# JuliaMolSim/Molly.jl

Hardware: AMD Instinct MI355X
Metric: ns_per_day (higher is better)
Workload: dtype f32; 1 GPU; 1M-atom LJ fluid (argon, rho=21.1/nm3), cubic PBC, DistanceCutoff 1.0 nm, r_list 1.2 nm, dt 2 fs, VelocityVerlet, remove_CM_motion=1; integrator=vv, n_atoms=1000000, rebuild_every=10, parallelism=single domain, block_atoms=256, j_split=2, pairs_half_list=75841147

## Files before the change

molly.jl_amd/csrc/engine.hip:

```cpp
#include <algorithm>
#include <chrono>
#include <cstddef>
#include <cstdlib>
#include <cstring>
#include <limits>
#include <memory>
#include <new>
#include <string>
#include <vector>

#include <unistd.h>

#include "bonded.h"
#include "stochastic.h"
#include "constraints.h"
#include "virtual_sites.h"
#include "pme.h"
#include "step_fused.h"
#include "hilbert.h"
#include "kernels.h"
#include "list_policy.h"
#include "replan.h"
#include "halo_step.h"
#include "forces_launch.h"
// ... 102 lines not shown
        MHIP_HIP(hipEventRecord(ev[st][used[st]].second, s));
        if (++used[st] >= 8192) resolve(s);
    }
    void resolve(hipStream_t s) {
        MHIP_HIP(hipStreamSynchronize(s));
        for (int st = 0; st < NS; ++st) {
            for (size_t k = 0; k < used[st]; ++k) { float t = 0; MHIP_HIP(hipEventSynchronize(ev[st][k].second)); MHIP_HIP(hipEventElapsedTime(&t, ev[st][k].first, ev[st][k].second)); ms[st] += t; ++calls[st]; }
            used[st] = 0;
        }
    }
    void reset() { for (int st = 0; st < NS; ++st) { used[st] = 0; ms[st] = 0; calls[st] = 0; } }
    void reserve(int st, size_t n) { while (ev[st].size() < n) add(st); }
    void add(int st) { Event a, b; a.make(); b.make(); ev[st].emplace_back(std::move(a), std::move(b)); }
};

static int env_int(const char* name, int dflt) { const char* v = std::getenv(name); return v && *v ? std::atoi(v) : dflt; }


template <class T> class Engine final : public EngineBase {
    using T4 = typename Vec<T>::T4;
    using T2 = typename Vec<T>::T2;

    mhip_config cfg;
    GridP<T> G;
    InterP<T> I;
    int ljm = LJ_OFF, coulm = MHIP_COUL_NONE;
    int64_t cap, n_owned, n_ghost, n_tot;
    Stream stream;
    int device = 0;

    DBuf<T4> pos[2], vel[2], frc[2]; DBuf<T2> lj[2]; DBuf<int32_t> orig[2]; DBuf<int32_t> inv;
    int cur = 0;
    DBuf<uint32_t> key_in, key_out, cell_rank; DBuf<int32_t> idx_in, perm, cell_cnt, cell_start; DBuf<unsigned char> cub_tmp;
    bool hilbert_ok = true;
    DBuf<int32_t> xl_start; DBuf<uint32_t> xl_list; bool has_exc = false; int xl_span = 0; int64_t n_special = 0;
    static constexpr int X_CAP = 32;
    static constexpr int MAX_THREADS = BlockLimits<T>::max_threads;
    int BI = 256, JS = 1, n_blocks = 0, T_cap = 0, R_cap = 0, C_cap = 0, max_tile = 0, max_rows = 0;
    int ljm_base = LJ_OFF;
    int eshift = 0;
    bool scaled_entries_off = false;
    int want_eshift() const {
        return (!scaled_entries_off && std::is_same<T, float>::value && ljm == LJ_DIST_UNIFORM && coulm == MHIP_COUL_NONE && n_special == 0 && !tri_mode && !G.no_list) ? ESHIFT_SCALED : 0;
    }
    int slot_cap() const { return ((want_eshift() ? SLOT_MAX_SCALED : TILE_SLOT_MAX) - 1) & ~3; }
    DBuf<int32_t> tile_idx, tile_cnt, wave_rows; DBuf<uint2> nbr; DBuf<T4> blk_center;
    DBuf<int32_t> wave_rows_in, tile_idx_in, tile_cnt_in, rows_x, tile_idx_x, tile_cnt_x; DBuf<uint2> nbr_in, nbr_x; DBuf<T4> pos_snap; DBuf<float> blk_disp2; int max_tile_in = 0;
    bool inner_valid = false, prune_disp_exceeded = false;
    DBuf<uint16_t> cnt_in, cnt_outer; bool cnt_outer_valid = false;
    DBuf<uint2> nbr_gs; DBuf<int32_t> rows_gs; DBuf<T4> frc_parts; int64_t gs_list_id = -1;
    bool inner_is_outer = false; const bool adopt_env = env_int("MOLLYHIP_ADOPT_OUTER", 1) != 0; int64_t n_adopted = 0;
    const int gs_env = env_int("MOLLYHIP_GROUP_SPLIT", -1);
    int gs_groups() const {
        if (!std::is_same<T, float>::value || ljm != LJ_DIST || !(coulm == MHIP_COUL_REACTION_FIELD || (coulm == MHIP_COUL_EWALD_DIRECT && I.approx_erfc))) return 0;
        if (!dual || tri_mode || n_ghost > 0 || G.no_list || gs_env == 0) return 0;
        const int want = gs_env > 0 ? gs_env : 4;
        if (want != 4 || JS % want != 0 || BI * (JS / want) != 256) return 0;
        if (gs_env < 0 && (int64_t)n_blocks * JS * (BI / WAVE) > 2 * 4096) return 0;
        if ((int64_t)n_blocks * want > 16384) return 0;
        return want;
    }
    DBuf<int32_t> blk_ghost, blk_ghost_in; bool ghost_flags_ok = false, ghost_flags_in_ok = false;
    bool interior_done = false;
    int64_t pass_step = 0;
    DBuf<T4> pos_snap_in;
    ListPolicy lp = [] { ListPolicy p; p.inner_skin_fixed = env_int("MOLLYHIP_INNER_SKIN_FIXED", 0) != 0; return p; }();
// ... 26 lines not shown
    DBuf<T> stage_a, stage_b; DBuf<int32_t> stage_i;
    Bonded<T> bonded;
    Pme<T> pme; double pc_sum = 0, pc_abs2_sum = 0; bool pc_valid = false;
    DBuf<T4> frc_side; const T4* pend_a = nullptr;

    bool stale = true, minimg = false, params_set = false, state_set = false, frc_valid = false;
    bool coords_moved = false, export_needs_search = false; int64_t n_set_state_refresh = 0;
    int64_t last_build_step = std::numeric_limits<int64_t>::min();
    int64_t n_rebuilds = 0, n_force_calls = 0, n_gs_passes = 0; double last_rebuild_ms = 0;
    PassPlan last_plan;
    Prof prof;
    const bool trace_on = env_int("MOLLYHIP_DEBUG", 0) >= 2;
    const bool debug_on = env_int("MOLLYHIP_DEBUG", 0) == 1 || env_int("MOLLYHIP_DEBUG", 0) >= 3;
    void tr(const char* what) {
        if (!trace_on) return;
        (void)hipStreamSynchronize(stream);
        std::fprintf(stderr, "[mhip %d] %s (n_owned %lld n_ghost %lld BI %d JS %d T_cap %d R_cap %d)\n", (int)getpid(), what, (long long)n_owned, (long long)n_ghost, BI, JS, T_cap, R_cap);
        std::fflush(stderr);
    }

  public:
    explicit Engine(const mhip_config& c) : cfg(c) {
        cap = c.n_atoms; n_owned = cap; n_ghost = 0; n_tot = cap;
        if (cap <= 0) throw ApiError{MHIP_ERR_INVALID, "n_atoms must be positive"};
        if (cap > (int64_t)1 << 30) throw ApiError{MHIP_ERR_INVALID, "n_atoms too large for int32 indexing"};
        int ndev = 0;
        if (hipGetDeviceCount(&ndev) != hipSuccess || ndev <= 0) throw ApiError{MHIP_ERR_NO_DEVICE, "no HIP device visible (libmollyhip has no CPU fallback)"};
        device = c.device_id;
        if (device < 0 || device >= ndev) throw ApiError{MHIP_ERR_INVALID, "device_id out of range"};
        MHIP_HIP(hipSetDevice(device));
        stream.create(hipStreamNonBlocking);
        setup_inter(); setup_grid();
        for (int k = 0; k < 2; ++k) { pos[k].reserve(cap); vel[k].reserve(cap); frc[k].reserve(cap); lj[k].reserve(cap); orig[k].reserve(cap); }
        inv.reserve(cap); key_in.reserve(cap); key_out.reserve(cap); idx_in.reserve(cap); perm.reserve(cap);
        flags.reserve(N_FLAGS); red_out.reserve(8); vcm.reserve(4); cm_step.reserve(2 * 4 * 1024);
        h_flags.make(N_FLAGS); h_red.make(8);
        for (int k = 0; k < 2; ++k) { MHIP_HIP(hipMemsetAsync(pos[k].p, 0, cap * sizeof(T4), stream)); MHIP_HIP(hipMemsetAsync(vel[k].p, 0, cap * sizeof(T4), stream)); MHIP_HIP(hipMemsetAsync(frc[k].p, 0, cap * sizeof(T4), stream)); MHIP_HIP(hipMemsetAsync(lj[k].p, 0, cap * sizeof(T2), stream)); }
        std::vector<int32_t> iota(cap); for (int64_t i = 0; i < cap; ++i) iota[i] = (int32_t)i;
        MHIP_HIP(hipMemcpyAsync(orig[0].p, iota.data(), cap * sizeof(int32_t), hipMemcpyHostToDevice, stream));
        MHIP_HIP(hipMemcpyAsync(inv.p, iota.data(), cap * sizeof(int32_t), hipMemcpyHostToDevice, stream));
        MHIP_HIP(hipStreamSynchronize(stream));
        size_t tb = 0; MHIP_HIP(sort_pairs_u32(nullptr, tb, key_in.p, key_out.p, idx_in.p, perm.p, (int)cap, 32, stream));
        size_t tb2 = 0; MHIP_HIP(exclusive_sum_i32(nullptr, tb2, cell_cnt.p, cell_start.p, 2 * G.ncell + 1, stream));
        cub_tmp.reserve(std::max(tb, tb2) + 256);
        choose_blocking();
    }
    ~Engine() override {
        (void)hipSetDevice(device);
        if (stream) (void)hipStreamSynchronize(stream);
    }

  private:
    void setup_inter() {
        const mhip_interactions& p = cfg.inter;
        std::memset(&I, 0, sizeof(I));
        I.lj = p.lj_enabled; I.lj_cut = p.lj_cutoff_kind; I.lj_rc = T(p.lj_rc); I.lj_rc2 = I.lj_rc * I.lj_rc; I.lj_ra = T(p.lj_ra); I.lj_w = T(p.lj_weight_special);
        I.coul = p.coul_kind; I.coul_cut = p.coul_cutoff_kind; I.c_rc = T(p.coul_rc); I.c_rc2 = I.c_rc * I.c_rc; I.c_ra = T(p.coul_ra);
        I.ke = T(p.coul_ke); I.c_w = T(p.coul_weight_special); I.alpha = T(p.ewald_alpha); I.approx_erfc = p.ewald_approx_erfc;
        I.two_over_sqrt_pi = T(2) / std::sqrt(T(M_PI));
        if (p.lj_cutoff_kind < 0 || p.lj_cutoff_kind > 5 || p.coul_cutoff_kind < 0 || p.coul_cutoff_kind > 5 || p.coul_kind < 0 || p.coul_kind > 3)
            throw ApiError{MHIP_ERR_INVALID, "unknown cutoff / coulomb kind"};
        if (p.coul_kind == MHIP_COUL_REACTION_FIELD) {
            T rc = I.c_rc, rc3 = rc * rc * rc, e = T(p.rf_dielectric);
            if (std::isinf(p.rf_dielectric)) { I.krf = T(1) / (T(2) * rc3); I.crf = T(3) * (T(1) / (T(2) * rc)); }
            else { I.krf = (T(1) / rc3) * (e - T(1)) / (T(2) * e + T(1)); I.crf = (T(1) / rc) * (T(3) * e) / (T(2) * e + T(1)); }
        }
        ljm = !p.lj_enabled ? LJ_OFF : (p.lj_cutoff_kind == MHIP_CUTOFF_DISTANCE ? LJ_DIST : LJ_GENERIC);
// ... 182 lines not shown
        if (!pending_cm.mode()) return;
        hipLaunchKernelGGL(k_shift_vel<T>, dim3(std::min(cdiv(n_owned, 256), 1024)), dim3(256), 0, stream, n_owned, vel[cur].p, (const T*)vcm.p,
                           pending_cm.parts_arg(), pending_cm.n, vs_on ? (const int32_t*)orig[cur].p : nullptr, (const uint8_t*)vs_flag.p);
        pending_cm.none();
    }

    const T* to_device(const void* host_or_dev, size_t count, int mem_kind, DBuf<T>& stage) {
        if (!host_or_dev) return nullptr;
        if (mem_kind == MHIP_MEM_DEVICE) return (const T*)host_or_dev;
        stage.reserve(count);
        MHIP_HIP(hipMemcpyAsync(stage.p, host_or_dev, count * sizeof(T), hipMemcpyHostToDevice, stream));
        return stage.p;
    }

    void rebuild(int64_t step_n) {
        try { rebuild_impl(step_n); }
        catch (const ApiError& e) {
            if (e.code != MHIP_ERR_CAPACITY || !dual) throw;
            if (n_ghost > 0 || ghost_margin > 0 || host_prune) dual_disabled = true;
            else if (lp.outer_margin > 0.06) ++margin_halvings; else if (!margin_zero) margin_zero = true; else dual_disabled = true;
            if (debug_on) std::fprintf(stderr, "[mhip] dual list %s (capacity): %s\n", dual_disabled ? "off" : (margin_zero ? "without outer margin" : "margin halved"), e.msg.c_str());
            regrid();
            rebuild(step_n);
        }
    }

    void rebuild_impl(int64_t step_n) {
        lp.next_check_step = -1;
        const int sub_bits = (ilog2(2 * G.ncell + 1) + 1 + 6 <= 32) ? 6 : 0;
        if (!params_set || !state_set) throw ApiError{MHIP_ERR_STATE, "set_atoms and set_state must be called before forces"};
        auto t0 = std::chrono::steady_clock::now();
        const int o = cur, n = 1 - cur;
        const int ncell2 = 2 * G.ncell + 1;
        prof.begin(3, stream);
        const int nb256 = cdiv(n_tot, 256);
        MHIP_HIP(hipMemsetAsync(cell_cnt.p, 0, (size_t)ncell2 * sizeof(int32_t), stream));
        tr("k_cell_keys");
        hipLaunchKernelGGL(k_cell_keys<T>, dim3(nb256), dim3(256), 0, stream, n_tot, n_owned, (const T4*)pos[o].p, (const int32_t*)inv.p,
                           (const uint32_t*)cell_rank.p, key_in.p, idx_in.p, cell_cnt.p, G, sub_bits);
        tr("sort_pairs");
        size_t tb = cub_tmp.n;
        MHIP_HIP(sort_pairs_u32(cub_tmp.p, tb, key_in.p, key_out.p, idx_in.p, perm.p, (int)n_tot, std::min(32, ilog2(2 * G.ncell + 1) + 1 + sub_bits), stream));
        tb = cub_tmp.n;
        MHIP_HIP(exclusive_sum_i32(cub_tmp.p, tb, cell_cnt.p, cell_start.p, ncell2, stream));
        tr("k_permute");
        hipLaunchKernelGGL(k_permute<T>, dim3(nb256), dim3(256), 0, stream, n_tot, (const int32_t*)perm.p, (const T4*)pos[o].p, (const T4*)vel[o].p,
                           (const T4*)frc[o].p, (const T2*)lj[o].p, (const int32_t*)orig[o].p, pos[n].p, vel[n].p, frc[n].p, lj[n].p, orig[n].p, inv.p);
        prof.end(3, stream);
        cur = n;
        if (n_ghost > 0 && has_exc) throw ApiError{MHIP_ERR_UNSUPPORTED, "exclusion lists with ghost atoms are not supported"};
        if (tri_mode && !tri_grid && n_tot + 8 > TILE_SLOT_MAX) throw ApiError{MHIP_ERR_UNSUPPORTED, "a TriclinicBoundary whose cell heights allow no cell grid (fewer than 6 cells of r_list/2 on every axis) is limited to 32 759 atoms"};

        for (int attempt = 0; attempt < 12; ++attempt) {
            n_blocks = cdiv(n_owned, BI);
            bool walk = !G.no_list && (!tri_mode || tri_grid);
            size_t lds = build_lds_bytes(T_cap, BI, C_cap, walk);
            if (walk && !tri_grid && lds > (size_t)MAX_LDS_BYTES) { walk = false; lds = build_lds_bytes(T_cap, BI, C_cap, false); }
            if (lds > (size_t)MAX_LDS_BYTES) {
                if (BI > 64) { BI /= 2; JS = std::min(JS * 2, MAX_THREADS / BI); estimate_capacities(); continue; }
                throw ApiError{MHIP_ERR_CAPACITY, "neighbourhood tile of one 64-atom block does not fit the 160 KiB LDS (r_list too large for this density): T_cap " + std::to_string(T_cap) +
                               " C_cap " + std::to_string(C_cap) + " bytes " + std::to_string(lds)};
            }
            tile_idx.reserve((size_t)n_blocks * T_cap); tile_cnt.reserve(n_blocks); wave_rows.reserve((size_t)n_blocks * JS * (BI / WAVE));
            nbr.reserve((size_t)n_blocks * JS * R_cap * BI); blk_center.reserve(n_blocks);
            MHIP_HIP(hipMemsetAsync(flags.p, 0, N_FLAGS * sizeof(int32_t), stream));
            BuildArgs<T> A;
            A.G = G; A.n_owned = n_owned; A.n_tot = n_tot; A.BI = BI; A.BI_shift = ilog2(BI); A.JS = JS; A.T_cap = T_cap; A.R_cap = R_cap; A.C_cap = C_cap;
            A.pos = pos[cur].p; A.orig = orig[cur].p; A.cell_start = cell_start.p; A.cell_rank = cell_rank.p;
            A.xl_start = has_exc ? xl_start.p : nullptr; A.xl_list = xl_list.p; A.xl_span = xl_span; A.X_cap = X_CAP;
            A.tile_idx = tile_idx.p; A.tile_cnt = tile_cnt.p; A.nbr = nbr.p; A.wave_rows = wave_rows.p; A.blk_center = blk_center.p; A.flags = flags.p;
            A.margin = G.no_list ? T(0) : G.r_list * T(1e-3);
            A.approx = dual ? 1 : 0;
            A.walk = walk ? 1 : 0;
            A.eshift = eshift = want_eshift();
            A.cnt_out = nullptr; cnt_outer_valid = false;
            A.dbg = stamps_begin((size_t)n_blocks * 16 * 8);
            if (gs_groups() > 0 && adopt_env) { cnt_outer.reserve((size_t)n_blocks * JS * BI); A.cnt_out = cnt_outer.p; cnt_outer_valid = true; }
            prof.begin(1, stream);
            tr("k_build");
            auto go = [&](auto kern) { set_lds_limit(kern, lds); hipLaunchKernelGGL(kern, dim3(n_blocks), dim3(BI * JS), lds, stream, A); };
            if (A.walk && !A.xl_start) { if (A.approx) go(k_build<T, true, true, false>); else go(k_build<T, true, false, false>); }
            else if (A.walk) { if (A.approx) go(k_build<T, true, true>); else go(k_build<T, true, false>); }
            else { if (A.approx) go(k_build<T, false, true>); else go(k_build<T, false, false>); }
            hipLaunchKernelGGL(k_build_summary, dim3(std::min(64, cdiv(n_blocks * JS * (BI / WAVE), 256))), dim3(256), 0, stream, n_blocks, n_blocks * JS * (BI / WAVE), R_cap, (const int32_t*)tile_cnt.p, wave_rows.p, (const float*)nullptr, flags.p);
            prof.end(1, stream);
            MHIP_HIP(hipGetLastError());
            MHIP_HIP(hipMemcpyAsync(h_flags, flags.p, N_FLAGS * sizeof(int32_t), hipMemcpyDeviceToHost, stream));
            MHIP_HIP(hipStreamSynchronize(stream));
            if (A.dbg) stamps_dump(".build", (size_t)n_blocks * 16 * 8);
            int ovf = h_flags[FLAG_OVERFLOW];
            if (!ovf) break;
            if (ovf & OVF_SLOT) {
                if (eshift) { scaled_entries_off = true; estimate_capacities(); continue; }
                if (BI > 64) { BI /= 2; JS = std::min(JS * 2, MAX_THREADS / BI); estimate_capacities(); continue; }
                throw ApiError{MHIP_ERR_CAPACITY, "more atoms within r_list of one 64-atom block than a 16-bit list entry can name"};
            }
            if (ovf & OVF_BOXCELLS) {
                if (h_flags[FLAG_MAX_CELLS] <= MAX_BOX_CELLS) { C_cap = std::min<int>(MAX_BOX_CELLS, (int)(h_flags[FLAG_MAX_CELLS] * 1.1) + 8); continue; }
                if (BI > 64) { BI /= 2; JS = std::min(JS * 2, MAX_THREADS / BI); estimate_capacities(); continue; }
                throw ApiError{MHIP_ERR_CAPACITY, "block neighbourhood spans more than 8192 cells"};
            }
            if (ovf & OVF_TILE) T_cap = std::min<int>(slot_cap(), (((int)(h_flags[FLAG_MAX_TILE] * 1.15) + 32) + 3) & ~3);
            if (ovf & OVF_ROWS) R_cap = (int)(h_flags[FLAG_MAX_ROWS] * 1.2) + 4;
            if (attempt == 11) throw ApiError{MHIP_ERR_CAPACITY, "neighbour structures did not converge"};
        }
        minimg = h_flags[FLAG_MINIMG] != 0;
        max_tile = h_flags[FLAG_MAX_TILE]; max_rows = h_flags[FLAG_MAX_ROWS]; total_rows = outer_rows = h_flags[FLAG_TOTAL_ROWS];
        last_plan = PassPlan{}; plan_tile(last_plan, pass_shape(false, 0, false, PassReq{}), max_tile);
        throw_capacity(last_plan);
        red_part.reserve(std::max<size_t>(7 * (size_t)n_blocks, 4 * (size_t)cdiv(n_owned, 256)) + 8);
        bonded.on_reorder();
        ++n_outer; lp.last_outer_step = step_n;
        if (dual) {
            pos_snap.reserve(cap);
            MHIP_HIP(hipMemcpyAsync(pos_snap.p, pos[cur].p, (size_t)n_tot * sizeof(T4), hipMemcpyDeviceToDevice, stream));
            inner_valid = false; inner_is_outer = false; prune_disp_exceeded = false; ghost_flags_in_ok = false;
            if (lp.cur_dt > 0 && lp.skin_in < lp.skin && !host_prune) {
                (void)max_disp2_since(pos_snap);
                const double drift = lp.drift_ahead(0.0, 1, rebuild_every());
                if (lp.grow_inner_skin(drift, n_ghost > 0)) inner_skin_grown(drift);
            }
        }
        if (lazy_single) {
            pos_snap_in.reserve(cap);
// ... 2259 lines not shown
```

molly.jl_amd/csrc/kernels.h:

```cpp
#pragma once
#include <type_traits>
#include "pass_plan.h"
#include "physics.h"
#include "halo_xfer.h"
#include "philox.h"
#include "thermostat_step.h"

namespace mhip {

enum { FLAG_MINIMG = 0, FLAG_OVERFLOW = 1, FLAG_MAX_TILE = 2, FLAG_MAX_ROWS = 3, FLAG_NAN = 4, FLAG_TOTAL_ROWS = 5, FLAG_MAX_CELLS = 6, FLAG_MAX_DISP2 = 7, FLAG_MAX_V2 = 8, N_FLAGS = 10 };
enum { OVF_TILE = 1, OVF_ROWS = 2, OVF_BOXCELLS = 4, OVF_SLOT = 8 };

constexpr int MAX_BOX_CELLS = 8192;
constexpr uint32_t XL_EXCLUDED = 1u << 30, XL_SPECIAL = 1u << 31, XL_INDEX = (1u << 30) - 1u;

constexpr int SLOT_MAX_SCALED = 16383;
__host__ __device__ inline uint32_t entry_slot(uint32_t e, int sh) { return sh ? (e >> sh) : (e & 0x7fffu); }
__host__ __device__ inline uint32_t entry_special(uint32_t e, int sh) { return sh ? 0u : (e >> 15); }
__host__ __device__ inline uint32_t make_entry(uint32_t slot, uint32_t sp, int sh) { return sh ? (slot << sh) : (slot | (sp << 15)); }

template <class T> __device__ inline int cell_coord(T x, int d, const GridP<T>& G) {
    T rel = G.periodic[d] ? x : x - G.origin[d];
    int c = (int)M<T>::floor(rel * G.inv_cs[d]);
    return min(max(c, 0), G.nc[d] - 1);
}

extern "C" __device__ int mhip_writelane_i32(int src, int lane, int old) __asm("llvm.amdgcn.writelane.i32");
__device__ inline void mask_to_lane(int& lo, int& hi, unsigned long long mask, int dst) {
    lo = mhip_writelane_i32((int)(uint32_t)mask, dst, lo);
    hi = mhip_writelane_i32((int)(uint32_t)(mask >> 32), dst, hi);
}
__device__ inline float lane_bcast(float v, int src) { return __int_as_float(__builtin_amdgcn_readlane(__float_as_int(v), src)); }
__device__ inline double lane_bcast(double v, int src) {
    long long b = __double_as_longlong(v);
    int lo = __builtin_amdgcn_readlane((int)(b & 0xffffffffll), src), hi = __builtin_amdgcn_readlane((int)(b >> 32), src);
    return __longlong_as_double(((long long)hi << 32) | (unsigned int)lo);
}

template <class T> __device__ inline T wave_max(T v) {
#pragma unroll
    for (int o = 32; o > 0; o >>= 1) { T u = __shfl_xor(v, o, 64); v = u > v ? u : v; }
    return v;
}

// ... 101 lines not shown

template <class T>
__global__ void k_scatter_params(int64_t n_tot, const int32_t* __restrict__ inv, const T* q, const T* sig, const T* eps,
                                 const T* mass, const T* lam, typename Vec<T>::T4* pos, typename Vec<T>::T4* vel,
                                 typename Vec<T>::T2* lj) {
    int64_t o = blockIdx.x * (int64_t)blockDim.x + threadIdx.x;
    if (o >= n_tot) return;
    int s = inv[o];
    pos[s].w = q ? q[o] : T(0);
    T sg = sig ? sig[o] : T(0), ep = eps ? eps[o] : T(0);
    if (lam && lam[o] == T(0)) { sg = T(0); ep = T(0); }
    lj[s] = make2<T>(sg, ep);
    vel[s].w = mass ? mass[o] : T(1);
}

template <class T>
__global__ void k_gather_state(int64_t n, const int32_t* __restrict__ inv, const typename Vec<T>::T4* __restrict__ src, T* out) {
    int64_t o = blockIdx.x * (int64_t)blockDim.x + threadIdx.x;
    if (o >= n) return;
    auto p = src[inv[o]];
    out[3 * o] = p.x; out[3 * o + 1] = p.y; out[3 * o + 2] = p.z;
}

template <class T>
__global__ void k_export_forces(int64_t n_owned, const int32_t* __restrict__ orig, const typename Vec<T>::T4* __restrict__ frc, T* out, int accumulate) {
    int64_t s = blockIdx.x * (int64_t)blockDim.x + threadIdx.x;
    if (s >= n_owned) return;
    int o = orig[s];
    auto f = frc[s];
    if (accumulate) { out[3 * o] += f.x; out[3 * o + 1] += f.y; out[3 * o + 2] += f.z; }
    else { out[3 * o] = f.x; out[3 * o + 1] = f.y; out[3 * o + 2] = f.z; }
}

template <class T>
__global__ void k_cell_keys(int64_t n_tot, int64_t n_owned, const typename Vec<T>::T4* __restrict__ pos, const int32_t* __restrict__ inv,
                            const uint32_t* __restrict__ cell_rank, uint32_t* key, int32_t* idx, int32_t* cell_cnt, GridP<T> G, int sub_bits) {
    int64_t o = blockIdx.x * (int64_t)blockDim.x + threadIdx.x;
    if (o >= n_tot) return;
    int s = inv[o];
    auto p = pos[s];
    int cc[3]; cell_coords(p.x, p.y, p.z, G, cc);
    uint32_t k = cell_rank[(cc[2] * G.nc[1] + cc[1]) * G.nc[0] + cc[0]];
    if (o >= n_owned) k += (uint32_t)G.ncell;
    uint32_t sub = 0;
    if (sub_bits && !G.tri_grid) {
        const T xyz[3] = {p.x, p.y, p.z};
#pragma unroll
        for (int d = 0; d < 3; ++d) {
            const T rel = (G.periodic[d] ? xyz[d] : xyz[d] - G.origin[d]) * G.inv_cs[d] - T(cc[d]);
            const int q = min(max((int)(rel * T(4)), 0), 3);
            sub |= (uint32_t)(q & 1) << d | (uint32_t)(q >> 1) << (3 + d);
        }
    }
    key[o] = (k << sub_bits) | sub; idx[o] = s;
    atomicAdd(&cell_cnt[k], 1);
}

template <class T>
__global__ void k_permute(int64_t n_tot, const int32_t* __restrict__ perm, const typename Vec<T>::T4* __restrict__ pos_o,
                          const typename Vec<T>::T4* __restrict__ vel_o, const typename Vec<T>::T4* __restrict__ frc_o,
                          const typename Vec<T>::T2* __restrict__ lj_o, const int32_t* __restrict__ orig_o,
                          typename Vec<T>::T4* pos_n, typename Vec<T>::T4* vel_n, typename Vec<T>::T4* frc_n,
                          typename Vec<T>::T2* lj_n, int32_t* orig_n, int32_t* inv) {
    int64_t s = blockIdx.x * (int64_t)blockDim.x + threadIdx.x;
    if (s >= n_tot) return;
    int so = perm[s];
    pos_n[s] = pos_o[so]; vel_n[s] = vel_o[so]; frc_n[s] = frc_o[so]; lj_n[s] = lj_o[so];
    int o = orig_o[so];
    orig_n[s] = o; inv[o] = (int32_t)s;
}

template <class T> struct BuildArgs {
    GridP<T> G;
    int64_t n_owned, n_tot;
    int BI, BI_shift, JS;
    int T_cap, R_cap, C_cap;
    const typename Vec<T>::T4* pos;
    const int32_t* orig;
    const int32_t* cell_start;
    const uint32_t* cell_rank;
    const int32_t* xl_start;
    const uint32_t* xl_list;
    int xl_span;
    int X_cap;
    int32_t* tile_idx;
    int32_t* tile_cnt;
// ... 9 lines not shown
    unsigned long long* dbg;
};

__device__ inline int block_excl_scan(int32_t* a, int n, int32_t* part, int tid, int nthr) {
    int per = (n + nthr - 1) / nthr, q0 = min(tid * per, n), q1 = min(q0 + per, n);
    int sum = 0;
    for (int q = q0; q < q1; ++q) sum += a[q];
    part[tid] = sum;
    __syncthreads();
    if (tid < WAVE) {
        int run = 0;
        for (int base = 0; base < nthr; base += WAVE) {
            int v = (base + tid < nthr) ? part[base + tid] : 0, x = v;
#pragma unroll
            for (int o = 1; o < WAVE; o <<= 1) { int u = __shfl_up(x, o, WAVE); if (tid >= o) x += u; }
            if (base + tid < nthr) part[base + tid] = run + x - v;
            run += __shfl(x, WAVE - 1, WAVE);
        }
        if (tid == 0) a[n] = run;
    }
    __syncthreads();
    int run = part[tid];
    for (int q = q0; q < q1; ++q) { int v = a[q]; a[q] = run; run += v; }
    __syncthreads();
    return a[n];
}

template <class T> struct BlockLimits { static constexpr int max_threads = sizeof(T) == 8 ? 512 : 1024; };

template <class T, bool WALK, bool APPROX, bool XL = true>
__global__ void __launch_bounds__(BlockLimits<T>::max_threads) k_build(BuildArgs<T> A) {
    using T4 = typename Vec<T>::T4;
    extern __shared__ __align__(32) unsigned char smem[];
    const GridP<T>& G = A.G;
    const int b = blockIdx.x, tid = threadIdx.x, nthr = blockDim.x, lane = tid & 63, wv_all = tid >> 6, NW_ALL = nthr >> 6;
    const int li = tid & (A.BI - 1), js = tid >> A.BI_shift;
    const int wv = li >> 6, NW = A.BI >> 6;
#if MHIP_STAMPS
    if (A.dbg && lane == 0) { unsigned long long* d = A.dbg + ((size_t)b * NW_ALL + wv_all) * 8; d[0] = wall_clock64(); }
#endif
    float* t_x = reinterpret_cast<float*>(smem);
    float* t_y = t_x + A.T_cap;
    float* t_z = t_y + A.T_cap;
    int32_t* t_orig = reinterpret_cast<int32_t*>(t_z + A.T_cap);
    int32_t* c_raw = t_orig + ((XL && A.xl_start) ? A.T_cap : 0);
    auto t_pos = [&](int t) { return make_float4(t_x[t], t_y[t], t_z[t], 0.f); };
    int32_t* c_rank = c_raw + (A.C_cap + 1);
    int32_t* part = c_rank + A.C_cap + 1;
    uint32_t* x_part = reinterpret_cast<uint32_t*>(part + nthr);
    int32_t* t_off = reinterpret_cast<int32_t*>(x_part + (A.xl_start ? A.X_cap * A.BI : 0));
    __shared__ T s_sub[4][6];
    __shared__ T s_ctr[3], s_half[3];
    __shared__ int s_boxlo[3], s_boxlen[3], s_full[3], s_exact, s_wtot[4 * 16];
    __shared__ int s_self[256];

    const int64_t si = (int64_t)b * A.BI + li;
    const bool valid = si < A.n_owned;
    T4 pi = A.pos[valid ? si : (int64_t)b * A.BI];
    T my[3] = {pi.x, pi.y, pi.z};
    T mu[3] = {pi.x, pi.y, pi.z};
    if (G.tri_grid) { T sf[3]; frac_coords(my[0], my[1], my[2], G, sf); mu[0] = sf[0] * G.hgt[0]; mu[1] = sf[1] * G.hgt[1]; mu[2] = sf[2] * G.hgt[2]; }
    {
        T mn[3] = {mu[0], mu[1], mu[2]}, mx[3] = {mu[0], mu[1], mu[2]};
#pragma unroll
        for (int o = 32; o > 0; o >>= 1)
#pragma unroll
// ... 238 lines not shown
            }
            if (!far || (unsigned)(oj - oi + A.xl_span) > (unsigned)(2 * A.xl_span)) return 0;
            uint32_t hit = 0;
            for (int k = 0; k < nxl; ++k) {
                const uint32_t e = k < A.X_cap ? x_part[k * A.BI + li] : A.xl_list[xl0 + k];
                hit = ((e & XL_INDEX) == (uint32_t)oj) ? e : hit;
            }
            return (hit & XL_EXCLUDED) ? -1 : (int)(hit >> 31);
        };
#if MHIP_STAMPS
        if (A.dbg && XL && A.xl_start) { int x = nxl; for (int o = 32; o > 0; o >>= 1) x += __shfl_xor(x, o, WAVE); if (lane == 0) A.dbg[((size_t)b * NW_ALL + wv_all) * 8 + 6] = (unsigned long long)x; }
#endif
        const Loc3 my_lc = localise3(my[0], my[1], my[2]);
        const float ml[3] = {(float)my_lc.l0, (float)my_lc.l1, (float)my_lc.l2};
        const float rl2 = G.no_list ? 3.0e38f : (float)G.r_list2;
        const float band_lo = rl2 * (1.0f - 1e-4f), band_hi = G.no_list ? 3.0e38f : rl2 * (1.0f + 1e-4f);
        const float reach2f = G.no_list ? 3.0e38f : (float)reach2;
        float blo[3], bhi[3];
#pragma unroll
        for (int d = 0; d < 3; ++d) { blo[d] = (float)(s_sub[wv][d] - ctr[d]); bhi[d] = (float)(s_sub[wv][3 + d] - ctr[d]); }
        const unsigned long long valid_mask = __ballot(valid);
        const uint32_t self_t = valid ? (uint32_t)s_self[li] : 0xffffffffu;
        if (WALK && !exact_only) {
            const bool js_pow2 = (A.JS & (A.JS - 1)) == 0;
            if (valid) {
                int qc[3], lo[3], hi[3], mycell[3];
                cell_coords(my[0], my[1], my[2], G, mycell);
#pragma unroll
                for (int d = 0; d < 3; ++d) {
                    int q = mycell[d] - s_boxlo[d];
                    if (G.periodic[d]) { if (q < 0) q += G.nc[d]; else if (q >= G.nc[d]) q -= G.nc[d]; }
                    qc[d] = q; lo[d] = max(q - G.stencil[d], 0); hi[d] = min(q + G.stencil[d], s_boxlen[d] - 1);
                }
                for (int qz = lo[2]; qz <= hi[2]; ++qz) for (int qy = lo[1]; qy <= hi[1]; ++qy) {
                    const int row = (qz * ly + qy) * lx;
                    const int t0 = t_off[row + lo[0]], t1 = t_off[row + hi[0] + 1];
                    int t = t0 + (js_pow2 ? ((js - t0) & (A.JS - 1)) : ((js - t0) % A.JS + A.JS) % A.JS);
                    auto consider = [&](int tc, const float4 pl) {
                        const float dx = pl.x - ml[0], dy = pl.y - ml[1], dz = pl.z - ml[2];
                        const float r2 = dx * dx + dy * dy + dz * dz;
                        bool in = APPROX ? r2 <= band_hi : r2 < band_lo;
                        if (!APPROX && !in && r2 <= band_hi) {
                            T4 pj = A.pos[A.tile_idx[(int64_t)b * A.T_cap + tc]];
                            T ex, ey, ez;
                            min_image_exact<T>(my[0], my[1], my[2], pj.x, pj.y, pj.z, G, ex, ey, ez);
                            in = norm2_exact(ex, ey, ez) <= G.r_list2;
                        }
                        if (!in || (uint32_t)tc == self_t) return;
                        uint32_t sp = 0;
                        const int oj = (XL && nxl > 0) ? t_orig[tc] : 0;
                        if constexpr (XL) {
                            if (nxl > 0) { const int v = exception_of(oj); if (v < 0) return; sp = (uint32_t)v; }
                        }
                        emit(make_entry((uint32_t)tc, sp, A.eshift));
                    };
                    const int last = t1 - 1;
                    if constexpr (APPROX && !XL) {
                        typedef float v2f __attribute__((ext_vector_type(2)));
                        const v2f mx2 = {ml[0], ml[0]}, my2 = {ml[1], ml[1]}, mz2 = {ml[2], ml[2]};
                        for (; t < t1; t += 4 * A.JS) {
                            const int ta = t, tb = t + A.JS, tc = t + 2 * A.JS, td = t + 3 * A.JS;
                            const int ib = min(tb, last), ic = min(tc, last), id = min(td, last);
                            const v2f dx0 = (v2f){t_x[ta], t_x[ib]} - mx2, dy0 = (v2f){t_y[ta], t_y[ib]} - my2, dz0 = (v2f){t_z[ta], t_z[ib]} - mz2;
                            const v2f dx1 = (v2f){t_x[ic], t_x[id]} - mx2, dy1 = (v2f){t_y[ic], t_y[id]} - my2, dz1 = (v2f){t_z[ic], t_z[id]} - mz2;
                            const v2f r20 = __builtin_elementwise_fma(dz0, dz0, __builtin_elementwise_fma(dy0, dy0, dx0 * dx0));
                            const v2f r21 = __builtin_elementwise_fma(dz1, dz1, __builtin_elementwise_fma(dy1, dy1, dx1 * dx1));
                            const bool ka = r20.x <= band_hi && (uint32_t)ta != self_t;
                            const bool kb = r20.y <= band_hi && (uint32_t)tb != self_t && tb < t1;
                            const bool kc = r21.x <= band_hi && (uint32_t)tc != self_t && tc < t1;
                            const bool kd = r21.y <= band_hi && (uint32_t)td != self_t && td < t1;
                            emit4(make_entry((uint32_t)ta, 0u, A.eshift), make_entry((uint32_t)ib, 0u, A.eshift), make_entry((uint32_t)ic, 0u, A.eshift), make_entry((uint32_t)id, 0u, A.eshift), ka, kb, kc, kd);
                        }
                    } else {
                    for (; t < t1; t += 4 * A.JS) {
                        const int ta = t, tb = t + A.JS, tc = t + 2 * A.JS, td = t + 3 * A.JS;
                        const float4 pa = t_pos(ta), pb = t_pos(min(tb, last)), pc = t_pos(min(tc, last)), pd = t_pos(min(td, last));
                        consider(ta, pa);
                        if (tb < t1) consider(tb, pb);
                        if (tc < t1) consider(tc, pc);
                        if (td < t1) consider(td, pd);
                    }
                    }
                }
                (void)qc;
            }
        } else {
        const int nwords = (tile_n + 64 * A.JS - 1) / (64 * A.JS);
        for (int w = 0; w < nwords; ++w) {
            const int jl = ((w << 6) + lane) * A.JS + js;
            float4 pl = make_float4(0.f, 0.f, 0.f, 0.f); bool near = false;
            T4 px = make4<T>(T(0), T(0), T(0), T(0));
            if (jl < tile_n) {
                pl = t_pos(jl);
                if (exact_only) { near = true; px = A.pos[A.tile_idx[(int64_t)b * A.T_cap + jl]]; }
                else {
                    float pc[3] = {pl.x, pl.y, pl.z}, acc = 0.f;
#pragma unroll
                    for (int d = 0; d < 3; ++d) { float e = blo[d] - pc[d]; float f = pc[d] - bhi[d]; e = e > f ? e : f; e = e > 0.f ? e : 0.f; acc += e * e; }
                    near = acc <= reach2f;
                }
            }
            if (__ballot(near) == 0ull) continue;
            int mine_lo = 0, mine_hi = 0;
            if (!exact_only) {
                float gmn[3] = {near ? pl.x : 3.0e38f, near ? pl.y : 3.0e38f, near ? pl.z : 3.0e38f};
                float gmx[3] = {near ? pl.x : -3.0e38f, near ? pl.y : -3.0e38f, near ? pl.z : -3.0e38f};
#pragma unroll
                for (int o = 32; o > 0; o >>= 1)
#pragma unroll
                    for (int d = 0; d < 3; ++d) { gmn[d] = fminf(gmn[d], __shfl_xor(gmn[d], o, WAVE)); gmx[d] = fmaxf(gmx[d], __shfl_xor(gmx[d], o, WAVE)); }
                float acc = 0.f;
#pragma unroll
                for (int d = 0; d < 3; ++d) { float e = gmn[d] - ml[d]; float f = ml[d] - gmx[d]; e = e > f ? e : f; e = e > 0.f ? e : 0.f; acc += e * e; }
                unsigned long long im = __ballot(valid && acc <= reach2f);
                const float qx = near ? pl.x : __builtin_inff();
                if (APPROX) {
                    while (im) {
// ... 1479 lines not shown
```

Before: 1373 ns/day.

## Replace radix sort with atomic counting-sort and skip self check off own row

Adds a counting-sort path for the cell rebuild. Wave-aggregated atomics assign each atom an arrival slot in its cell bin, the records are scattered into cell groups, and each atom's rank inside its cell is computed by comparison so the permuted order stays deterministic. This path is used when the system has 64 atoms per cell or fewer. If any bin exceeds the cap, an overflow flag makes the build kernel exit early and the rebuild reruns with the radix sort. Separately, the approximate list build now walks stencil rows so that the self-index comparison only runs on the atom's own row. The intent is to cut the radix-sort passes and some per-candidate work, at the cost of extra buffers and an intra-cell rank loop that grows with the square of the cell occupancy.

```diff
diff --git a/molly.jl_amd/csrc/cell_sort.h b/molly.jl_amd/csrc/cell_sort.h
--- /dev/null
+++ b/molly.jl_amd/csrc/cell_sort.h
@@ -0,0 +1,55 @@
+#pragma once
+#include <hip/hip_runtime.h>
+#include <stdint.h>
+
+namespace mhip {
+
+constexpr int CELL_SORT_MAX_BIN = 2048;
+
+__device__ inline void cell_sort_count(bool active, int64_t s, uint32_t bin, uint32_t sub, int32_t caller, int32_t* cell_cnt, uint4* rec,
+                                       int max_bin, int32_t* ovf_word, int ovf_bit) {
+    const int lane = (int)__lane_id();
+    const uint32_t key = active ? bin : 0xffffffffu;
+    const uint32_t prev = __shfl_up(key, 1);
+    const unsigned long long heads = __ballot(lane == 0 || key != prev);
+    const unsigned long long mine = (2ull << lane) - 1ull;
+    const int head = 63 - __clzll((long long)(heads & mine));
+    const unsigned long long later = heads & ~mine;
+    const int end = later ? __ffsll((long long)later) - 1 : 64;
+    int base = 0;
+    if (active && lane == head) base = atomicAdd(&cell_cnt[bin], end - head);
+    base = __shfl(base, head);
+    if (!active) return;
+    const int arrival = base + (lane - head);
+    if (arrival == max_bin) atomicOr(ovf_word, ovf_bit);
+    rec[s] = make_uint4((uint32_t)caller, sub, bin, (uint32_t)arrival);
+}
+
+template <class I>
+__global__ void k_cell_sort_scatter(I n, const uint4* __restrict__ rec, const int32_t* __restrict__ cell_start, uint4* grouped,
+                                    const int32_t* __restrict__ ovf_word, int ovf_bit) {
+    if (*ovf_word & ovf_bit) return;
+    const int64_t s = blockIdx.x * (int64_t)blockDim.x + threadIdx.x;
+    if (s >= n) return;
+    const uint4 r = rec[s];
+    grouped[(int64_t)cell_start[r.z] + r.w] = make_uint4(r.x, r.y, r.z, (uint32_t)s);
+}
+
+template <class Move>
+__global__ void k_cell_sort_rank(int64_t n, const uint4* __restrict__ grouped, const int32_t* __restrict__ cell_start,
+                                 const int32_t* __restrict__ ovf_word, int ovf_bit, Move move) {
+    if (*ovf_word & ovf_bit) return;
+    const int64_t p = blockIdx.x * (int64_t)blockDim.x + threadIdx.x;
+    if (p >= n) return;
+    const uint4 me = grouped[p];
+    const int lo = cell_start[me.z], hi = cell_start[me.z + 1];
+    const uint64_t w = (uint64_t)me.y << 32 | me.x;
+    const uint2* words = reinterpret_cast<const uint2*>(grouped);
+    auto below = [&](int q) { const uint2 o = words[2 * (int64_t)q]; return ((uint64_t)o.y << 32 | o.x) < w ? 1 : 0; };
+    int rank = 0, q = lo;
+    for (; q + 4 <= hi; q += 4) { const int a = below(q), b = below(q + 1), c = below(q + 2), d = below(q + 3); rank += (a + b) + (c + d); }
+    for (; q < hi; ++q) rank += below(q);
+    move((int64_t)lo + rank, (int64_t)me.w, (int32_t)me.x);
+}
+
+}
diff --git a/molly.jl_amd/csrc/engine.hip b/molly.jl_amd/csrc/engine.hip
--- a/molly.jl_amd/csrc/engine.hip
+++ b/molly.jl_amd/csrc/engine.hip
@@ -158,6 +158,7 @@
     DBuf<T4> pos[2], vel[2], frc[2]; DBuf<T2> lj[2]; DBuf<int32_t> orig[2]; DBuf<int32_t> inv;
     int cur = 0;
     DBuf<uint32_t> key_in, key_out, cell_rank; DBuf<int32_t> idx_in, perm, cell_cnt, cell_start; DBuf<unsigned char> cub_tmp;
+    DBuf<uint4> cs_rec, cs_grouped;
     bool hilbert_ok = true;
     DBuf<int32_t> xl_start; DBuf<uint32_t> xl_list; bool has_exc = false; int xl_span = 0; int64_t n_special = 0;
     static constexpr int X_CAP = 32;
@@ -250,7 +251,7 @@
         stream.create(hipStreamNonBlocking);
         setup_inter(); setup_grid();
         for (int k = 0; k < 2; ++k) { pos[k].reserve(cap); vel[k].reserve(cap); frc[k].reserve(cap); lj[k].reserve(cap); orig[k].reserve(cap); }
-        inv.reserve(cap); key_in.reserve(cap); key_out.reserve(cap); idx_in.reserve(cap); perm.reserve(cap);
+        inv.reserve(cap); key_in.reserve(cap); key_out.reserve(cap); idx_in.reserve(cap); perm.reserve(cap); cs_rec.reserve(cap); cs_grouped.reserve(cap);
         flags.reserve(N_FLAGS); red_out.reserve(8); vcm.reserve(4); cm_step.reserve(2 * 4 * 1024);
         h_flags.make(N_FLAGS); h_red.make(8);
         for (int k = 0; k < 2; ++k) { MHIP_HIP(hipMemsetAsync(pos[k].p, 0, cap * sizeof(T4), stream)); MHIP_HIP(hipMemsetAsync(vel[k].p, 0, cap * sizeof(T4), stream)); MHIP_HIP(hipMemsetAsync(frc[k].p, 0, cap * sizeof(T4), stream)); MHIP_HIP(hipMemsetAsync(lj[k].p, 0, cap * sizeof(T2), stream)); }
@@ -499,22 +500,48 @@
         auto t0 = std::chrono::steady_clock::now();
         const int o = cur, n = 1 - cur;
         const int ncell2 = 2 * G.ncell + 1;
-        prof.begin(3, stream);
         const int nb256 = cdiv(n_tot, 256);
-        MHIP_HIP(hipMemsetAsync(cell_cnt.p, 0, (size_t)ncell2 * sizeof(int32_t), stream));
-        tr("k_cell_keys");
-        hipLaunchKernelGGL(k_cell_keys<T>, dim3(nb256), dim3(256), 0, stream, n_tot, n_owned, (const T4*)pos[o].p, (const int32_t*)inv.p,
-                           (const uint32_t*)cell_rank.p, key_in.p, idx_in.p, cell_cnt.p, G, sub_bits);
-        tr("sort_pairs");
-        size_t tb = cub_tmp.n;
-        MHIP_HIP(sort_pairs_u32(cub_tmp.p, tb, key_in.p, key_out.p, idx_in.p, perm.p, (int)n_tot, std::min(32, ilog2(2 * G.ncell + 1) + 1 + sub_bits), stream));
-        tb = cub_tmp.n;
-        MHIP_HIP(exclusive_sum_i32(cub_tmp.p, tb, cell_cnt.p, cell_start.p, ncell2, stream));
-        tr("k_permute");
-        hipLaunchKernelGGL(k_permute<T>, dim3(nb256), dim3(256), 0, stream, n_tot, (const int32_t*)perm.p, (const T4*)pos[o].p, (const T4*)vel[o].p,
-                           (const T4*)frc[o].p, (const T2*)lj[o].p, (const int32_t*)orig[o].p, pos[n].p, vel[n].p, frc[n].p, lj[n].p, orig[n].p, inv.p);
-        prof.end(3, stream);
+        auto sort_stage = [&](bool radix) {
+            MHIP_HIP(hipMemsetAsync(flags.p, 0, N_FLAGS * sizeof(int32_t), stream));
+            prof.begin(3, stream);
+            MHIP_HIP(hipMemsetAsync(cell_cnt.p, 0, (size_t)ncell2 * sizeof(int32_t), stream));
+            size_t tb = cub_tmp.n;
+            if (radix) {
+                tr("k_cell_keys");
+                hipLaunchKernelGGL(k_cell_keys<T>, dim3(nb256), dim3(256), 0, stream, n_tot, n_owned, (const T4*)pos[o].p, (const int32_t*)inv.p,
+                                   (const uint32_t*)cell_rank.p, key_in.p, idx_in.p, cell_cnt.p, G, sub_bits);
+                tr("sort_pairs");
+                MHIP_HIP(sort_pairs_u32(cub_tmp.p, tb, key_in.p, key_out.p, idx_in.p, perm.p, (int)n_tot, std::min(32, ilog2(2 * G.ncell + 1) + 1 + sub_bits), stream));
+                tb = cub_tmp.n;
+                MHIP_HIP(exclusive_sum_i32(cub_tmp.p, tb, cell_cnt.p, cell_start.p, ncell2, stream));
+                tr("k_permute");
+                hipLaunchKernelGGL(k_permute<T>, dim3(nb256), dim3(256), 0, stream, n_tot, (const int32_t*)perm.p, (const T4*)pos[o].p, (const T4*)vel[o].p,
+                                   (const T4*)frc[o].p, (const T2*)lj[o].p, (const int32_t*)orig[o].p, pos[n].p, vel[n].p, frc[n].p, lj[n].p, orig[n].p, inv.p);
+            } else {
+                tr("k_cell_count");
+                hipLaunchKernelGGL(k_cell_count<T>, dim3(nb256), dim3(256), 0, stream, n_tot, n_owned, (const T4*)pos[o].p, (const int32_t*)orig[o].p,
+                                   (const uint32_t*)cell_rank.p, cell_cnt.p, cs_rec.p, G, sub_bits, CELL_SORT_MAX_BIN, flags.p);
+                MHIP_HIP(exclusive_sum_i32(cub_tmp.p, tb, cell_cnt.p, cell_start.p, ncell2, stream));
+                tr("k_cell_sort_rank");
+                hipLaunchKernelGGL(k_cell_sort_scatter<int64_t>, dim3(nb256), dim3(256), 0, stream, n_tot, (const uint4*)cs_rec.p, (const int32_t*)cell_start.p, cs_grouped.p,
+                                   (const int32_t*)(flags.p + FLAG_OVERFLOW), (int)OVF_SORT);
+                hipLaunchKernelGGL(k_cell_sort_rank<PermuteAtom<T>>, dim3(nb256), dim3(256), 0, stream, n_tot, (const uint4*)cs_grouped.p, (const int32_t*)cell_start.p,
+                                   (const int32_t*)(flags.p + FLAG_OVERFLOW), (int)OVF_SORT,
+                                   PermuteAtom<T>{pos[o].p, vel[o].p, frc[o].p, lj[o].p, pos[n].p, vel[n].p, frc[n].p, lj[n].p, orig[n].p, inv.p});
+            }
+            prof.end(3, stream);
+        };
+        sort_stage(n_tot > 64 * (int64_t)G.ncell);
         cur = n;
+        struct SortVerdict {
+            Engine* e; int o; bool pending = true;
+            ~SortVerdict() {
+                int32_t w = 0;
+                if (pending && hipMemcpyAsync(&w, e->flags.p + FLAG_OVERFLOW, sizeof w, hipMemcpyDeviceToHost, e->stream) == hipSuccess &&
+                    hipStreamSynchronize(e->stream) == hipSuccess && (w & OVF_SORT)) e->cur = o;
+            }
+        } verdict{this, o};
+        bool flags_clean = true;
         if (n_ghost > 0 && has_exc) throw ApiError{MHIP_ERR_UNSUPPORTED, "exclusion lists with ghost atoms are not supported"};
         if (tri_mode && !tri_grid && n_tot + 8 > TILE_SLOT_MAX) throw ApiError{MHIP_ERR_UNSUPPORTED, "a TriclinicBoundary whose cell heights allow no cell grid (fewer than 6 cells of r_list/2 on every axis) is limited to 32 759 atoms"};
 
@@ -530,7 +557,8 @@
             }
             tile_idx.reserve((size_t)n_blocks * T_cap); tile_cnt.reserve(n_blocks); wave_rows.reserve((size_t)n_blocks * JS * (BI / WAVE));
             nbr.reserve((size_t)n_blocks * JS * R_cap * BI); blk_center.reserve(n_blocks);
-            MHIP_HIP(hipMemsetAsync(flags.p, 0, N_FLAGS * sizeof(int32_t), stream));
+            if (!flags_clean) MHIP_HIP(hipMemsetAsync(flags.p, 0, N_FLAGS * sizeof(int32_t), stream));
+            flags_clean = false;
             BuildArgs<T> A;
             A.G = G; A.n_owned = n_owned; A.n_tot = n_tot; A.BI = BI; A.BI_shift = ilog2(BI); A.JS = JS; A.T_cap = T_cap; A.R_cap = R_cap; A.C_cap = C_cap;
             A.pos = pos[cur].p; A.orig = orig[cur].p; A.cell_start = cell_start.p; A.cell_rank = cell_rank.p;
@@ -556,7 +584,9 @@
             MHIP_HIP(hipStreamSynchronize(stream));
             if (A.dbg) stamps_dump(".build", (size_t)n_blocks * 16 * 8);
             int ovf = h_flags[FLAG_OVERFLOW];
+            verdict.pending = false;
             if (!ovf) break;
+            if (ovf & OVF_SORT) { sort_stage(true); flags_clean = true; continue; }
             if (ovf & OVF_SLOT) {
                 if (eshift) { scaled_entries_off = true; estimate_capacities(); continue; }
                 if (BI > 64) { BI /= 2; JS = std::min(JS * 2, MAX_THREADS / BI); estimate_capacities(); continue; }
diff --git a/molly.jl_amd/csrc/kernels.h b/molly.jl_amd/csrc/kernels.h
--- a/molly.jl_amd/csrc/kernels.h
+++ b/molly.jl_amd/csrc/kernels.h
@@ -5,11 +5,12 @@
 #include "halo_xfer.h"
 #include "philox.h"
 #include "thermostat_step.h"
+#include "cell_sort.h"
 
 namespace mhip {
 
 enum { FLAG_MINIMG = 0, FLAG_OVERFLOW = 1, FLAG_MAX_TILE = 2, FLAG_MAX_ROWS = 3, FLAG_NAN = 4, FLAG_TOTAL_ROWS = 5, FLAG_MAX_CELLS = 6, FLAG_MAX_DISP2 = 7, FLAG_MAX_V2 = 8, N_FLAGS = 10 };
-enum { OVF_TILE = 1, OVF_ROWS = 2, OVF_BOXCELLS = 4, OVF_SLOT = 8 };
+enum { OVF_TILE = 1, OVF_ROWS = 2, OVF_BOXCELLS = 4, OVF_SLOT = 8, OVF_SORT = 16 };
 
 constexpr int MAX_BOX_CELLS = 8192;
 constexpr uint32_t XL_EXCLUDED = 1u << 30, XL_SPECIAL = 1u << 31, XL_INDEX = (1u << 30) - 1u;
@@ -177,26 +178,51 @@
     else { out[3 * o] = f.x; out[3 * o + 1] = f.y; out[3 * o + 2] = f.z; }
 }
 
+template <class T, class V4>
+__device__ inline void cell_sort_key(const V4& p, int64_t o, int64_t n_owned, const uint32_t* __restrict__ cell_rank, const GridP<T>& G, int sub_bits,
+                                     uint32_t& k, uint32_t& sub) {
+    int cc[3]; cell_coords(p.x, p.y, p.z, G, cc);
+    k = cell_rank[(cc[2] * G.nc[1] + cc[1]) * G.nc[0] + cc[0]];
+    if (o >= n_owned) k += (uint32_t)G.ncell;
+    sub = 0;
+    if (sub_bits && !G.tri_grid) {
+        const T xyz[3] = {p.x, p.y, p.z};
+#pragma unroll
+        for (int d = 0; d < 3; ++d) {
+            const T rel = (G.periodic[d] ? xyz[d] : xyz[d] - G.origin[d]) * G.inv_cs[d] - T(cc[d]);
+            const int q = min(max((int)(rel * T(4)), 0), 3);
+            sub |= (uint32_t)(q & 1) << d | (uint32_t)(q >> 1) << (3 + d);
+        }
+    }
+}
+
+template <class T>
+__global__ void k_cell_count(int64_t n_tot, int64_t n_owned, const typename Vec<T>::T4* __restrict__ pos, const int32_t* __restrict__ orig,
+                             const uint32_t* __restrict__ cell_rank, int32_t* cell_cnt, uint4* rec, GridP<T> G, int sub_bits, int max_bin, int32_t* flags) {
+    int64_t s = blockIdx.x * (int64_t)blockDim.x + threadIdx.x;
+    const bool active = s < n_tot;
+    int o = 0; uint32_t k = 0, sub = 0;
+    if (active) { o = orig[s]; cell_sort_key(pos[s], (int64_t)o, n_owned, cell_rank, G, sub_bits, k, sub); }
+    cell_sort_count(active, s, k, sub, o, cell_cnt, rec, max_bin, &flags[FLAG_OVERFLOW], OVF_SORT);
+}
+
+template <class T> struct PermuteAtom {
+    const typename Vec<T>::T4* __restrict__ pos_o; const typename Vec<T>::T4* __restrict__ vel_o; const typename Vec<T>::T4* __restrict__ frc_o;
+    const typename Vec<T>::T2* __restrict__ lj_o;
+    typename Vec<T>::T4* pos_n; typename Vec<T>::T4* vel_n; typename Vec<T>::T4* frc_n; typename Vec<T>::T2* lj_n; int32_t* orig_n; int32_t* inv;
+    __device__ void operator()(int64_t s, int64_t so, int32_t o) const {
+        pos_n[s] = pos_o[so]; vel_n[s] = vel_o[so]; frc_n[s] = frc_o[so]; lj_n[s] = lj_o[so];
+        orig_n[s] = o; inv[o] = (int32_t)s;
+    }
+};
+
 template <class T>
 __global__ void k_cell_keys(int64_t n_tot, int64_t n_owned, const typename Vec<T>::T4* __restrict__ pos, const int32_t* __restrict__ inv,
                             const uint32_t* __restrict__ cell_rank, uint32_t* key, int32_t* idx, int32_t* cell_cnt, GridP<T> G, int sub_bits) {
     int64_t o = blockIdx.x * (int64_t)blockDim.x + threadIdx.x;
     if (o >= n_tot) return;
     int s = inv[o];
-    auto p = pos[s];
-    int cc[3]; cell_coords(p.x, p.y, p.z, G, cc);
-    uint32_t k = cell_rank[(cc[2] * G.nc[1] + cc[1]) * G.nc[0] + cc[0]];
-    if (o >= n_owned) k += (uint32_t)G.ncell;
-    uint32_t sub = 0;
-    if (sub_bits && !G.tri_grid) {
-        const T xyz[3] = {p.x, p.y, p.z};
-#pragma unroll
-        for (int d = 0; d < 3; ++d) {
-            const T rel = (G.periodic[d] ? xyz[d] : xyz[d] - G.origin[d]) * G.inv_cs[d] - T(cc[d]);
-            const int q = min(max((int)(rel * T(4)), 0), 3);
-            sub |= (uint32_t)(q & 1) << d | (uint32_t)(q >> 1) << (3 + d);
-        }
-    }
+    uint32_t k, sub; cell_sort_key(pos[s], o, n_owned, cell_rank, G, sub_bits, k, sub);
     key[o] = (k << sub_bits) | sub; idx[o] = s;
     atomicAdd(&cell_cnt[k], 1);
 }
@@ -272,6 +298,7 @@
 __global__ void __launch_bounds__(BlockLimits<T>::max_threads) k_build(BuildArgs<T> A) {
     using T4 = typename Vec<T>::T4;
     extern __shared__ __align__(32) unsigned char smem[];
+    if (A.flags[FLAG_OVERFLOW] & OVF_SORT) return;
     const GridP<T>& G = A.G;
     const int b = blockIdx.x, tid = threadIdx.x, nthr = blockDim.x, lane = tid & 63, wv_all = tid >> 6, NW_ALL = nthr >> 6;
     const int li = tid & (A.BI - 1), js = tid >> A.BI_shift;
@@ -576,7 +603,8 @@
                     if (G.periodic[d]) { if (q < 0) q += G.nc[d]; else if (q >= G.nc[d]) q -= G.nc[d]; }
                     qc[d] = q; lo[d] = max(q - G.stencil[d], 0); hi[d] = min(q + G.stencil[d], s_boxlen[d] - 1);
                 }
-                for (int qz = lo[2]; qz <= hi[2]; ++qz) for (int qy = lo[1]; qy <= hi[1]; ++qy) {
+                auto walk_row = [&](const int qz, const int qy, auto own_row) {
+                    constexpr bool OWN = decltype(own_row)::value;
                     const int row = (qz * ly + qy) * lx;
                     const int t0 = t_off[row + lo[0]], t1 = t_off[row + hi[0] + 1];
                     int t = t0 + (js_pow2 ? ((js - t0) & (A.JS - 1)) : ((js - t0) % A.JS + A.JS) % A.JS);
@@ -609,10 +637,10 @@
                             const v2f dx1 = (v2f){t_x[ic], t_x[id]} - mx2, dy1 = (v2f){t_y[ic], t_y[id]} - my2, dz1 = (v2f){t_z[ic], t_z[id]} - mz2;
                             const v2f r20 = __builtin_elementwise_fma(dz0, dz0, __builtin_elementwise_fma(dy0, dy0, dx0 * dx0));
                             const v2f r21 = __builtin_elementwise_fma(dz1, dz1, __builtin_elementwise_fma(dy1, dy1, dx1 * dx1));
-                            const bool ka = r20.x <= band_hi && (uint32_t)ta != self_t;
-                            const bool kb = r20.y <= band_hi && (uint32_t)tb != self_t && tb < t1;
-                            const bool kc = r21.x <= band_hi && (uint32_t)tc != self_t && tc < t1;
-                            const bool kd = r21.y <= band_hi && (uint32_t)td != self_t && td < t1;
+                            const bool ka = r20.x <= band_hi && (!OWN || (uint32_t)ta != self_t);
+                            const bool kb = r20.y <= band_hi && (!OWN || (uint32_t)tb != self_t) && tb < t1;
+                            const bool kc = r21.x <= band_hi && (!OWN || (uint32_t)tc != self_t) && tc < t1;
+                            const bool kd = r21.y <= band_hi && (!OWN || (uint32_t)td != self_t) && td < t1;
                             emit4(make_entry((uint32_t)ta, 0u, A.eshift), make_entry((uint32_t)ib, 0u, A.eshift), make_entry((uint32_t)ic, 0u, A.eshift), make_entry((uint32_t)id, 0u, A.eshift), ka, kb, kc, kd);
                         }
                     } else {
@@ -625,8 +653,16 @@
                         if (td < t1) consider(td, pd);
                     }
                     }
+                };
+                if constexpr (APPROX && !XL) {
+                    for (int dz = -G.stencil[2]; dz <= G.stencil[2]; ++dz) for (int dy = -G.stencil[1]; dy <= G.stencil[1]; ++dy) {
+                        const int qz = qc[2] + dz, qy = qc[1] + dy;
+                        if (qz < 0 || qz >= s_boxlen[2] || qy < 0 || qy >= s_boxlen[1]) continue;
+                        if (dz == 0 && dy == 0) walk_row(qz, qy, std::true_type{}); else walk_row(qz, qy, std::false_type{});
+                    }
+                } else {
+                    for (int qz = lo[2]; qz <= hi[2]; ++qz) for (int qy = lo[1]; qy <= hi[1]; ++qy) walk_row(qz, qy, std::true_type{});
                 }
-                (void)qc;
             }
         } else {
         const int nwords = (tile_n + 64 * A.JS - 1) / (64 * A.JS);
```

Measured after the change: 1402 ns/day (median of 6 runs). 1.02x the previous value.
